# penn-graphics-research/DOT

Measured on AMD Instinct MI355X. Metric: ms_per_time_step, lower is better.
Workload: dtype f64; 1 GPU; bar17K_twist; nV=17315, nT=86058, energy=SNH, subdomains=32, script=twist, parallelism=32 subdomains on 1 GPU

## Files before the change

### dot_amd/csrc/dotmi_api.hip

```cpp
#include "dotmi_handle.hpp"

extern "C" {

int dotmi_set_state(dotmi_handle *h, const double *x, const double *v, const double *x_n)
{
    if (!h || !x || !v) return DOTMI_E_INVALID;
    HIPCHECK(h, hipSetDevice(h->device));
    if (resolve_refresh(h) == DOTMI_E_DEVICE) return DOTMI_E_DEVICE;
    const size_t bytes = sizeof(double) * h->n;
    HIPCHECK(h, hipMemcpyAsync(h->x, x, bytes, hipMemcpyHostToDevice, h->st));
    HIPCHECK(h, hipMemcpyAsync(h->v, v, bytes, hipMemcpyHostToDevice, h->st));
    HIPCHECK(h, hipMemcpyAsync(h->xn, x_n ? x_n : x, bytes, hipMemcpyHostToDevice, h->st));
    HIPCHECK(h, hipStreamSynchronize(h->st));
    std::vector<double> xt(h->n);
    const double *xn_h = x_n ? x_n : x;
    for (int i = 0; i < h->nV; ++i)
        for (int d = 0; d < 3; ++d) {
            const int k = 3 * i + d;
            xt[k] = h->fixed[i] ? xn_h[k] : xn_h[k] + (v[k] * h->dt + h->gdtsq[d]);
        }
    HIPCHECK(h, hipMemcpy(h->xt, xt.data(), bytes, hipMemcpyHostToDevice));
    return 0;
}

// ... 37 lines not shown
    else HIPCHECK(h, hipEventSynchronize(h->evDir));
    memcpy(h->dposPinned, pos, sizeof(double) * 3 * n);
    HIPCHECK(h, hipMemcpyAsync(h->dpos, h->dposPinned, sizeof(double) * 3 * n, hipMemcpyHostToDevice, h->st));
    HIPCHECK(h, hipEventRecord(h->evDir, h->st));
    launch_scatter_rows(n, h->didx, h->dpos, h->x, h->st);
    return 0;
}

int dotmi_refix(dotmi_handle *h, const uint8_t *fixed)
{
    if (!h || !fixed) return DOTMI_E_INVALID;
    HIPCHECK(h, hipSetDevice(h->device));
    if (resolve_refresh(h) == DOTMI_E_DEVICE) return DOTMI_E_DEVICE;
    h->fixed.assign(fixed, fixed + h->nV);
    HIPCHECK(h, hipMemcpy(h->M.fixed, fixed, h->nV, hipMemcpyHostToDevice));
    if (h->pd) return pd_factor(h);
    return refactor(h, h->x, nullptr, nullptr);
}

double dotmi_target_gres(const dotmi_handle *h) { return h ? h->targetGRes : 0.0; }

int dotmi_last_iter_log(const dotmi_handle *h, int32_t cap, double *alpha, double *E, double *g2)
{
    if (!h) return DOTMI_E_INVALID;
    if (h->logPending > 0) {
        dotmi_handle *hm = const_cast<dotmi_handle *>(h);
        const int nlog = h->logPending;
        hm->logPending = 0;
        hm->log_alpha.resize(nlog);
        hm->log_E.resize(nlog);
        hm->log_g2.resize(nlog);
        if (hipSetDevice(h->device) != hipSuccess ||
            hipMemcpy(hm->log_alpha.data(), h->dlog, sizeof(double) * nlog, hipMemcpyDeviceToHost) != hipSuccess ||
// ... 558 lines not shown
```

### dot_amd/csrc/dotmi_create.hip

```cpp
#include "dotmi_handle.hpp"
#include "block_plan.hpp"

namespace dotmi {
std::string g_create_error;
}

namespace dotmi {

void host_features(dotmi_handle *h)
{
    const int nV = h->nV, nT = h->nT;
    h->A.assign((size_t)9 * nT, 0.0);
    h->vol.assign(nT, 0.0);
    h->mass.assign(nV, 0.0);
    for (int e = 0; e < nT; ++e) {
        const int *t = &h->T[4 * e];
        const double *p0 = &h->Xrest[3 * t[0]], *p1 = &h->Xrest[3 * t[1]], *p2 = &h->Xrest[3 * t[2]],
                     *p3 = &h->Xrest[3 * t[3]];
        Mat3 X0;
        for (int i = 0; i < 3; ++i) {
            X0.m[i][0] = p1[i] - p0[i];
            X0.m[i][1] = p2[i] - p0[i];
            X0.m[i][2] = p3[i] - p0[i];
        }
// ... 743 lines not shown
    if (!owner || H.nPatches == 0) return 0;
    for (int p = 0; p < H.nPatches; ++p) {
        const uint16_t *cp = &H.c_ptr[(size_t)p * (H.PO + 1)];
        for (int lv = 0; lv < H.po_cnt[p]; ++lv) {
            const int v = H.pv_gid[(size_t)p * H.PV + lv];
            owner[v] = p;
            if (runlen) runlen[v] = cp[lv + 1] - cp[lv];
        }
    }
    if (elem) std::copy(H.elem.begin(), H.elem.end(), elem);
    if (eown)
        for (size_t s = 0; s < H.eown.size(); ++s) eown[s] = H.eown[s];
    return 0;
}

static int plan_tile_schedule_impl(int32_t nt, const uint8_t *live, const uint8_t *pattern, const int32_t *c0, int32_t eager_min,
                                   int32_t eager_chunk, int64_t *tasks, int64_t *prods, int64_t *n_tasks, int64_t *n_prods,
                                   int64_t *n_levels, int64_t *storage, int64_t *scratch_base, int64_t *row_off, int32_t *row_ld,
                                   const uint8_t *leaf_tile, const int32_t *c0m, const int32_t *ntm, int64_t *row_off_m,
                                   int32_t *row_ld_m)
{
    if (nt < 1 || !live || !pattern || !c0 || !n_tasks || !n_prods) return DOTMI_E_INVALID;
    std::vector<long long> rtOff(nt, -1);
    std::vector<int> rtLd(nt, 0), rtC0(nt, 0);
    long long tot = 0;
    for (int j = 0; j < nt; ++j) {
        if (!live[j]) continue;
        rtC0[j] = 64 * c0[j];
        rtLd[j] = 64 * (j + 1) - rtC0[j];
        rtOff[j] = tot;
// ... 602 lines not shown
        return DOTMI_E_INVALID;
    }
    h->devLoop = !h->gsdd && !h->newton && !h->pd && !h->hi && !(h->flags & (DOTMI_FLAG_HOST_LOOP | DOTMI_FLAG_TIME_PHASES));
    h->earlyBs = h->devLoop && h->tune.earlyBs != 0 &&
                 (h->P.mt_ptr != nullptr || h->P.splitMerge);
    if (h->owner && !(h->earlyBs && h->tune.fuseDir)) {
        h->err = "DOTMI_FLAG_OWNER_EXCHANGE needs the device loop's early order with the fused direction kernel";
        return DOTMI_E_INVALID;
    }
    if (h->earlyBs && h->tune.fuseStep && (!h->shardElems || h->owner)) h->PT.wgCap = h->PTspec.wgCap = 512;
    h->vpFits = false;
    if (h->earlyBs && !h->dist && h->world == 1 && h->tune.fuseStep && h->tune.fuseDir && h->tune.vertexPatches != 0 &&
        (h->mat == DOTMI_ENERGY_SNH || h->tune.vertexPatches > 0) &&
        h->P.ntiles - h->P.ntilesWide + h->P.nquad > 0 && !(h->flags & (DOTMI_FLAG_GSDD | DOTMI_FLAG_NEWTON | DOTMI_FLAG_NEWTON_PCG | DOTMI_FLAG_HOST_LOOP))) {
        const HostVPatches HV = build_vpatches(h->nV, h->nT, h->T.data(), h->Xrest.data(), 512, 85);
        const size_t shm = sizeof(double) * ((size_t)3 * HV.PV + (size_t)3 * HV.RUN) + 2 * (size_t)((HV.PO + 1 + 3) & ~3);
        if (HV.nPatches > 0 && HV.nPatches <= 512 && HV.nPatches <= ELEM_NB_MAX && shm <= 64 * 1024 && HV.PO + 1 <= 256) {
            if (int rc = upload_vpatches(h, HV, h->VP, h->smVP)) return rc;
            h->vpFits = true;
            if (h->tune.fuseLog)
                fprintf(stderr, "dotmi: vertex patches: %d patches, %.2f x the elements, up to %d owned / %d touched vertices, runs %d, %zu B LDS\n",
                        HV.nPatches, (double)h->VP.nSlotsUsed / std::max(1, h->nT), HV.PO, HV.PV, HV.RUN, shm);
        }
    }
    return 0;
}

static int alloc_loop_state(dotmi_handle *h)
{
    if (h->dist) {
        if (int rc = dalloc(h, &h->zstage, (size_t)h->n)) return rc;
        HIPCHECK(h, hipMemsetAsync(h->zstage, 0, sizeof(double) * h->n, h->st));
    }
    if (h->earlyBs) {
        if (int rc = dalloc(h, &h->u_old, (size_t)h->n)) return rc;
        for (int sl = 0; sl <= h->hist; ++sl) {
            if (int rc = dalloc(h, &h->MY[sl], (size_t)h->n)) return rc;
            if (int rc = dalloc(h, &h->HS[sl], (size_t)h->n)) return rc;
        }
    }
    h->logCap = std::min(h->iterCap, 10001) + 1;
    h->kindCap = 4096;
    HIPCHECK(h, hipHostMalloc((void **)&h->h_ctl, sizeof(DevLoop)));
    HIPCHECK(h, hipHostMalloc((void **)&h->h_flags, sizeof(int) * 4));
    HIPCHECK(h, hipMalloc((void **)&h->ctl, sizeof(DevLoop)));
    h->allocs.push_back(h->ctl);
    if (int rc = dalloc(h, &h->dlog, (size_t)3 * h->logCap)) return rc;
// ... 139 lines not shown
```

### dot_amd/csrc/dotmi_devloop.hip

```cpp
#include "dotmi_handle.hpp"

namespace dotmi {

struct Slot {
    int nb = 0;
    const double *spart = nullptr;
    const double *ctlE = nullptr;
};

static int slot_direction(dotmi_handle *h, Slot &s)
{
    if (h->specNow) {
        StepArgs sa{h->p, h->partS, h->alpha_dev, h->alphaMin};
        launch_dirstep(h->M, h->PTspec, h->mat, h->dtSq, h->xt, h->partE, &s.nb, h->Hval, h->z, h->partCT, h->p, h->Hp, h->partS, h->st,
                       h->ctl, sa);
    } else if (h->owner) {
        launch_spmv_zp(h->M, h->HvalOwn, h->z, h->partGC, h->p, h->Hp, h->partS, h->st, h->ctl, 0, -1, h->heldMask, h->ownMask,
                       h->held());
    } else if (h->tune.fuseDir) {
        launch_spmv_zp(h->M, h->Hval, h->z, h->dist ? h->partC : h->partCT, h->p, h->Hp, h->partS, h->st, h->ctl,
                       h->shardElems ? h->v0 : 0, h->shardElems ? h->v1 : -1, nullptr, nullptr, VList(), !h->dist, h->partST);
    } else {
        LbfgsArgs L0;
        memset(&L0, 0, sizeof(L0));
// ... 180 lines not shown
    C.iterCap = h->iterCap;
    C.hist = h->hist;
    C.tol = h->targetGRes;
    C.dtSq = h->dtSq;
    C.x_cur = h->x;
    C.x_trial = h->x_trial;
    C.g_cur = h->g;
    C.g_trial = h->g_trial;
    for (int s = 0; s <= h->hist; ++s) {
        C.S[s] = h->S[s];
        C.Y[s] = h->Y[s];
        C.MY[s] = h->MY[s];
        C.HS[s] = h->HS[s];
    }
    C.u_old = h->u_old;
    devloop_resolve(C);
    C.holdEnable = h->tune.earlyHold ? 1 : 0;
    memcpy(C.predHist, h->predState, sizeof(int) * 2);
    memcpy(&C.predCtr[0][0], h->predState + 2, sizeof(int) * 8);
    memcpy(C.pairCtr, h->pairState, sizeof(int) * 3);
    C.log_alpha = h->dlog;
    C.log_E = h->dlog + h->logCap;
    C.log_g2 = h->dlog + 2 * (size_t)h->logCap;
    C.slot_kind = h->dkind;
    C.logCap = h->logCap;
    C.kindCap = h->kindCap;
    volatile int *flags = h->h_flags;
    flags[0] = 0;
    flags[1] = 0;
    C.notifyFrom = std::max(0, std::min(h->prevSlots - 3, h->prevSlots * 3 / 4));
// ... 222 lines not shown
```

### dot_amd/csrc/dotmi_handle.hpp

```cpp
#pragma once
#include <hip/hip_runtime.h>
#include <rccl/rccl.h>

#include <algorithm>
#include <chrono>
#include <cmath>
#include <cstdio>
#include <cstdlib>
#include <cstring>
#include <functional>
#include <string>
#include <unordered_map>
#include <vector>

#include "../../include/dotmi.h"
#include "dotmi_internal.hpp"
#include "elem_math.hpp"
#include "partition.hpp"
#include "patches.hpp"
#include "vpatches.hpp"


namespace dotmi {

// ... 31 lines not shown
    int tileGroups = -1;
    int tileHfill = 1;
    int tileEagerMin = 0;
    int fastDiag = 1;
    int tileFlow = -1;
    int tileFlowWaitMs = 2000;
    int tileEagerMinRmul = -1;
    bool tileEagerMinRmulByUser = false;
    bool fuseDir = true;
    bool fuseStep = true;
    int pairTrials = -1;
    int vertexPatches = -1;
    int specStep = 0;
    bool earlyHold = true;
    int earlyBs = 2;
    static int geti(const char *name, int dflt)
    {
        const char *ev = getenv(name);
        return ev ? atoi(ev) : dflt;
    }
    static Tuning from_env()
    {
        Tuning t;
        t.wavePacks = geti("DOTMI_WAVE_PACKS", 1) != 0;
        t.tilePasses = std::min(8, std::max(1, geti("DOTMI_TILE_PASSES", 4)));
        t.ndLevels = geti("DOTMI_ND_LEVELS", -1);
        if (t.ndLevels < -1) t.ndLevels = 0;
        t.ndMin = std::max(128, geti("DOTMI_ND_MIN", ND_MIN_SPLIT));
        t.ndMinByUser = getenv("DOTMI_ND_MIN") != nullptr;
        if (const char *ev = getenv("DOTMI_TILE_ROWS")) t.tileRows = std::min(64, std::max(8, atoi(ev) / 8 * 8));
// ... 11 lines not shown
        t.tileGroups = geti("DOTMI_TILE_GROUPS", -1);
        t.tileHfill = geti("DOTMI_TILE_HFILL", 1) != 0;
        t.tileEagerMin = std::max(0, geti("DOTMI_TILE_EAGER_MIN", 0));
        t.tileFlow = geti("DOTMI_TILE_FLOW", -1);
        t.fastDiag = geti("DOTMI_FAST_DIAG", 1);
        t.tileFlowWaitMs = std::max(1, geti("DOTMI_TILE_FLOW_WAIT_MS", 2000));
        t.tileEagerMinRmul = geti("DOTMI_TILE_EAGER_MIN_RMUL", -1);
        t.tileEagerMinRmulByUser = getenv("DOTMI_TILE_EAGER_MIN_RMUL") != nullptr;
        t.earlyBs = geti("DOTMI_EARLY_BACKSOLVE", 2) != 0 ? 2 : 0;
        t.earlyHold = geti("DOTMI_EARLY_HOLD", 1) != 0;
        t.pairTrials = geti("DOTMI_PAIR_TRIALS", -1);
        t.specStep = geti("DOTMI_SPEC_STEP", 0);
        t.vertexPatches = geti("DOTMI_VERTEX_PATCHES", -1);
        t.fuseStep = geti("DOTMI_FUSE_STEP", 1) != 0;
        t.fuseDir = geti("DOTMI_FUSE_DIR", 1) != 0;
        return t;
    }
};

struct dotmi_handle {
    Tuning tune;
#ifdef DOTMI_TEST_HOOKS
    int testIterDelta = 0;
    int testFailRefresh = 0, testRefreshCount = 0;
#endif
    int nV = 0, nT = 0, n = 0, mat = 0, hist = 5, iterCap = 10000;
    double dt = 0, dtSq = 0, grav[3] = {0, 0, 0}, gdtsq[3] = {0, 0, 0}, relTol = 1e-5, alphaMin = 0.1;
    double targetGRes = 0, density = 0;
    int device = 0, rank = 0, world = 1, flags = 0;
    bool dist = false;
// ... 48 lines not shown
    bool tileSplit = false;
    int predState[10] = {0, 0, 1, 1, 1, 1, 1, 1, 1, 1};
    int heldSlots = 0, heldRejected = 0;
    bool tileFlow = false;
    bool fastDiag = false;
    int *tdepPtr = nullptr, *tdepIdx = nullptr, *tdone = nullptr, *tnext = nullptr;
    int tileEpoch = 0, nTtasks = 0, tileFlowWg = 0;
    hipStream_t stDiag = nullptr;
    std::vector<hipEvent_t> tFork, tJoin;
    double tileFlops = 0;
    DevPatches PT, PTall;
    DevPatches PTspec;
    bool specFits = false;
    DevVPatches VP;
    bool vpFits = false, vpNow = false;
    struct SlotMap {
        int *elem = nullptr;
        size_t nSlots = 0;
        double *mu = nullptr, *lam = nullptr;
    };
    SlotMap smAll, smOwn, smSpec, smVP;
    int nOwnElem = 0, v0 = 0, v1 = 0;
    double *x = nullptr, *x_trial = nullptr, *xn = nullptr, *v = nullptr, *xt = nullptr;
    double *g = nullptr, *g_trial = nullptr, *p = nullptr, *q = nullptr, *z = nullptr, *Hp = nullptr;
    double *He = nullptr, *Hval = nullptr, *tmpn = nullptr;
    double *S[HIST_MAX + 1] = {nullptr}, *Y[HIST_MAX + 1] = {nullptr};
    bool refreshPending = false;
    double carryHess = 0, carryFact = 0;
    bool earlyBs = false;
    bool earlyNow = false;
// ... 209 lines not shown
```

### dot_amd/csrc/dotmi_internal.hpp

```cpp
#pragma once
#include <hip/hip_runtime.h>

#include "nd_layout.hpp"
#include "tile_factor.hpp"
#include <stdint.h>

namespace dotmi {

constexpr int HIST_MAX = 6;
inline int elem_wg_cap(int mat) { return mat == 1 ? 768 : 512; }
constexpr int NB_RED = 256;
constexpr int RED_K = 3 * HIST_MAX + 3;
constexpr int BS_WAVE = 256;
constexpr int BS_NARROW = 3072;
constexpr int BS_LONG = 5120;
constexpr int ELEM_NB_MAX = 8192;
constexpr int CHOL_NB = 64;

__host__ __device__ inline size_t hval_idx(int blk, int e) { return (size_t)(blk >> 3) * 72 + (size_t)(8 * e + (blk & 7)); }
inline size_t hval_size(int nnzb) { return (size_t)72 * (((size_t)nnzb + 7) / 8); }

struct DevMesh {
    int nV, nT, nTp;
    int4 *T;
// ... 9 lines not shown

struct DevPatches {
    int nPatches = 0, PE = 0, PV = 0, nSlots = 0, nElem = 0;
    int wgCap = 0;
    ushort4 *tl = nullptr;
    double *A = nullptr;
    double *mu = nullptr, *lam = nullptr, *vol = nullptr;
    double mu0 = 0.0, lam0 = 0.0;
    int *pv_gid = nullptr, *pv_slot = nullptr, *pv_cnt = nullptr;
    unsigned short *c_ptr = nullptr;
    ushort4 *epos = nullptr;
    int2 *pp_rng = nullptr;
    double *gpart = nullptr;
};

struct DevVPatches {
    int nPatches = 0, PE = 0, PV = 0, PO = 0, RUN = 0, nSlotsUsed = 0;
    ushort4 *tl = nullptr, *epos = nullptr;
    double *A = nullptr;
    double *vol = nullptr, *volE = nullptr;
    double *mu = nullptr, *lam = nullptr;
    double mu0 = 0.0, lam0 = 0.0;
    int *pv_gid = nullptr, *pv_cnt = nullptr, *po_cnt = nullptr;
    unsigned short *c_ptr = nullptr;
};
struct ElemVertArgs {
    const double *mass, *xt, *p, *hp;
    const double *spmv_partials;
    const uint8_t *fixed;
    const int *vp_ptr, *vp_off;
    double *rpad;
    double *partE, *partR, *alpha_out;
    double dtSq, alpha_min;
    const double *x0;
    double *g0;
};

struct RowTile {
    long long off;
    int ld, c0;
// ... 143 lines not shown
    int logCap, kindCap;
    int pairNew;
    int abortEpoch;
    int holdEnable, holdNext, holdVerdict;
    int redo;
    int heldSlots, heldRejected;
    int pairSlots, pairRedo;
    int pairCtr[3], pairPad;
    int predHist[2], predCtr[2][4];
    const double *specPartials;
    double alphaMin;
    int specSlots, specRedo, firstTrials, unitFirst;
    double *u_old, *MY[HIST_MAX + 1];
    double *HS[HIST_MAX + 1];
    double *s_new, *y_new, *hs_new;
    double *my_new;
    const double *Lmy[HIST_MAX], *Lhs[HIST_MAX];
};
template <class DL>
__host__ __device__ inline void devloop_resolve(DL &C)
{
    C.s_new = C.S[C.slot];
    C.y_new = C.Y[C.slot];
    C.hs_new = C.HS[C.slot];
    const int m = C.L.m;
    for (int i = 0; i < HIST_MAX; ++i) {
        C.Lmy[i] = i < m ? C.MY[C.order[i]] : nullptr;
        C.Lhs[i] = i < m ? C.HS[C.order[i]] : nullptr;
    }
    C.my_new = m > 0 ? C.MY[C.order[m - 1]] : nullptr;
}
struct VList {
    const int *v = nullptr;
    int n = 0;
};
struct CtlArgs {
    DevLoop *ctl;
    const double *partE, *partR, *alpha_dev;
    int *flags_host;
    int nbE;
    int init;
};

void launch_step_forward(int n, const double *x0, const double *p, double *x, const double *spmv_partials,
                         double alpha_host, int use_partials, double alpha_min, double *alpha_out,
// ... 166 lines not shown
```

### dot_amd/csrc/k_elemvert.hip

```cpp
#include "k_device.hpp"

namespace dotmi {

constexpr int EV_EPT = 2;

#ifdef K_PROFILE
__device__ long long g_evprof[512][8];
extern "C" int dotmi_debug_evprof(long long *out)
{
    return (int)hipMemcpyFromSymbol(out, HIP_SYMBOL(g_evprof), sizeof(long long) * 512 * 8);
}
#define EVSTAMP(i) do { if (threadIdx.x == 0 && blockIdx.x < 512) g_evprof[blockIdx.x][i] = wall_clock64(); } while (0)
#else
#define EVSTAMP(i) do { } while (0)
#endif

template <int MAT, bool PAIR>
__global__ __launch_bounds__(256) void elem_vertex_kernel(DevVPatches VP, ElemVertArgs a, const DevLoop *__restrict__ ctl)
{
    extern __shared__ double lds[];
    __shared__ double sm[4 * RED_K];
    __shared__ double sme[8];
    __shared__ double sh_alpha;
    const bool pairedLaunch = PAIR && a.alpha_min < 0.0;
    const double alphaMin = pairedLaunch ? -a.alpha_min : a.alpha_min;
    const bool second = pairedLaunch && (int)blockIdx.x >= VP.nPatches;
    const int tid = threadIdx.x, p = second ? (int)blockIdx.x - VP.nPatches : (int)blockIdx.x;
    long long t_start = 0;
#ifdef K_PROFILE
    t_start = wall_clock64();
#endif
    const double *__restrict__ x = a.x0;
    double *__restrict__ x_out = nullptr, *__restrict__ g_out = a.g0;
    const double *__restrict__ g_old = nullptr;
    double *__restrict__ s_new = nullptr, *__restrict__ y_new = nullptr, *__restrict__ hs_new = nullptr;
    const double *hs[HIST_MAX], *hy[HIST_MAX];
    int hm = 0, lphase = 1;
    double lalpha = 0.0;
    const bool loop = ctl != nullptr;
    if (loop) {
        const int status = ctl->status;
        lphase = ctl->phase;
        lalpha = ctl->alpha;
        x = ctl->x_cur;
        x_out = ctl->x_trial;
        g_out = ctl->g_trial;
        g_old = ctl->g_cur;
        s_new = ctl->s_new;
        y_new = ctl->y_new;
        hs_new = ctl->hs_new;
        hm = ctl->L.m;
#pragma unroll
        for (int i = 0; i < HIST_MAX; ++i) {
            hs[i] = ctl->L.s[i];
            hy[i] = ctl->L.y[i];
        }
        if (status != 0) return;
    }
#ifdef K_PROFILE
    if (threadIdx.x == 0 && blockIdx.x < 512) g_evprof[blockIdx.x][7] = t_start;
#endif
    EVSTAMP(0);
    double pgv[NB_RED / 64], pHpv[NB_RED / 64];
    const bool usePart = loop && lphase == 0;
    if (usePart && tid < 64) {
#pragma unroll
        for (int u = 0; u < NB_RED / 64; ++u) {
            pgv[u] = a.spmv_partials[tid + 64 * u];
            pHpv[u] = a.spmv_partials[NB_RED + tid + 64 * u];
        }
    }
    constexpr int PE = 256 * EV_EPT;
    double *xs = lds, *gs = lds + 3 * VP.PV;
    unsigned short *cptr = reinterpret_cast<unsigned short *>(gs + 3 * VP.RUN);
    const int nv = VP.pv_cnt[p], no = VP.po_cnt[p];
    const size_t vb = (size_t)p * VP.PV;
    const int gid = tid < VP.PV ? VP.pv_gid[vb + tid] : -1;
    const unsigned short cp_reg = tid <= VP.PO ? VP.c_ptr[(size_t)p * (VP.PO + 1) + tid] : (unsigned short)0;
    const int ov = tid / 3, od = tid - 3 * ov;
    const int ogid_raw = ov < VP.PV ? VP.pv_gid[vb + ov] : -1;
    const bool vlane = tid < 3 * no;
    const int ogid = vlane ? ogid_raw : -1;
    ushort4 tl[EV_EPT], ep[EV_EPT];
    double Ai[EV_EPT][9], mu_[EV_EPT], la_[EV_EPT], vo[EV_EPT], voE[EV_EPT];
    const size_t strideA = (size_t)VP.nPatches * PE;
#pragma unroll
    for (int u = 0; u < EV_EPT; ++u) {
        const size_t s = (size_t)p * PE + u * 256 + tid;
        tl[u] = VP.tl[s];
        ep[u] = VP.epos[s];
#pragma unroll
        for (int k = 0; k < 9; ++k) Ai[u][k] = VP.A[(size_t)k * strideA + s];
        mu_[u] = VP.mu ? VP.mu[s] : VP.mu0;
        la_[u] = VP.mu ? VP.lam[s] : VP.lam0;
        vo[u] = VP.vol[s];
        voE[u] = VP.volE[s];
    }
    double xv[3] = {0, 0, 0}, pv[3] = {0, 0, 0};
    if (gid >= 0) {
#pragma unroll
        for (int d = 0; d < 3; ++d) {
            xv[d] = x[3 * gid + d];
            if (loop) pv[d] = a.p[3 * gid + d];
        }
    }
    const int ok = 3 * ogid + od;
    bool fx = true;
    double gold = 0.0, pk = 0.0, hpk = 0.0, ms = 0.0, xt_own = 0.0, xtv[3] = {0, 0, 0}, si[HIST_MAX], yi[HIST_MAX];
    int cb = 0, ce = 0;
#pragma unroll
    for (int i = 0; i < HIST_MAX; ++i) si[i] = yi[i] = 0.0;
    if (vlane) {
        fx = a.fixed[ogid] != 0;
        ms = a.mass[ogid];
        xt_own = a.xt[ok];
        if (od == 0) {
#pragma unroll
            for (int d = 0; d < 3; ++d) xtv[d] = a.xt[3 * ogid + d];
        }
        cb = a.vp_ptr[ogid];
        ce = a.vp_ptr[ogid + 1];
        if (loop) {
            gold = g_old[ok];
            pk = a.p[ok];
            hpk = a.hp[ok];
#pragma unroll
            for (int i = 0; i < HIST_MAX; ++i) {
// ... 26 lines not shown
                    if (pairedLaunch) a.alpha_out[1] = pair ? al : 0.0;
                }
            } else {
                sh_alpha = al;
                if (p == 0 && loop) *a.alpha_out = al;
            }
        }
    }
    __syncthreads();
    const double alpha = sh_alpha;
    if (second && alpha < 0.0) return;
    EVSTAMP(2);
    if (gid >= 0) {
#pragma unroll
        for (int d = 0; d < 3; ++d) xs[3 * tid + d] = loop ? xv[d] + alpha * pv[d] : xv[d];
    }
    for (int lv = tid + 256; lv < nv; lv += 256) {
        const int g2 = VP.pv_gid[vb + lv];
#pragma unroll
        for (int d = 0; d < 3; ++d) xs[3 * lv + d] = loop ? x[3 * g2 + d] + alpha * a.p[3 * g2 + d] : x[3 * g2 + d];
    }
    __syncthreads();
    EVSTAMP(3);
    constexpr int VC = 4;
    int vof[VC];
#pragma unroll
    for (int c = 0; c < VC; ++c) vof[c] = (cb + c < ce) ? a.vp_off[cb + c] : 0;
    double acc = 0.0;
#pragma unroll
    for (int u = 0; u < EV_EPT; ++u) {
        if (tl[u].x == 0xFFFF) continue;
        const double *p0 = xs + 3 * tl[u].x, *p1 = xs + 3 * tl[u].y, *p2 = xs + 3 * tl[u].z, *p3 = xs + 3 * tl[u].w;
        Mat3 F;
#pragma unroll
        for (int r = 0; r < 3; ++r) {
            const double d0 = p1[r] - p0[r], d1 = p2[r] - p0[r], d2 = p3[r] - p0[r];
#pragma unroll
            for (int c = 0; c < 3; ++c) F.m[r][c] = d0 * Ai[u][c] + d1 * Ai[u][3 + c] + d2 * Ai[u][6 + c];
        }
        const double w = a.dtSq * vo[u];
        double P[3][3];
        if constexpr (MAT == 1) {
// ... 32 lines not shown
        for (int aa = 0; aa < 3; ++aa)
#pragma unroll
            for (int c = 0; c < 3; ++c)
                g[3 + 3 * aa + c] = Ai[u][3 * aa] * P[c][0] + Ai[u][3 * aa + 1] * P[c][1] + Ai[u][3 * aa + 2] * P[c][2];
#pragma unroll
        for (int c = 0; c < 3; ++c) g[c] = -g[3 + c] - g[6 + c] - g[9 + c];
        const int pkk[4] = {ep[u].x, ep[u].y, ep[u].z, ep[u].w};
#pragma unroll
        for (int k = 0; k < 4; ++k)
            if (pkk[k] != 0xFFFF && !second) {
                gs[pkk[k]] = g[3 * k];
                gs[VP.RUN + pkk[k]] = g[3 * k + 1];
                gs[2 * VP.RUN + pkk[k]] = g[3 * k + 2];
            }
    }
    __syncthreads();
    EVSTAMP(4);
    double st[RED_K];
#pragma unroll
    for (int j = 0; j < RED_K; ++j) st[j] = 0.0;
    double ine = 0.0;
    if (vlane && second) {
        if (od == 0) {
            const double dx = xs[3 * ov] - xtv[0], dy = xs[3 * ov + 1] - xtv[1], dz = xs[3 * ov + 2] - xtv[2];
            ine = (dx * dx + dy * dy + dz * dz) * ms / 2.0;
        }
    } else if (vlane) {
        const int kb = cptr[ov], ke = cptr[ov + 1];
        const double *run = gs + od * VP.RUN;
        double sum = 0.0;
        for (int k = kb; k < ke; k += 4) {
            const double w0 = run[k], w1 = k + 1 < ke ? run[k + 1] : 0.0, w2 = k + 2 < ke ? run[k + 2] : 0.0,
                         w3 = k + 3 < ke ? run[k + 3] : 0.0;
            sum += w0;
            if (k + 1 < ke) sum += w1;
            if (k + 2 < ke) sum += w2;
            if (k + 3 < ke) sum += w3;
        }
        const double xt_k = xs[3 * ov + od];
        const double g = fx ? 0.0 : sum + ms * (xt_k - xt_own);
        if (x_out) x_out[ok] = xt_k;
        g_out[ok] = g;
#pragma unroll
        for (int c = 0; c < VC; ++c)
            if (cb + c < ce) a.rpad[vof[c] + od] = -g;
        for (int c = cb + VC; c < ce; ++c) a.rpad[a.vp_off[c] + od] = -g;
        st[0] = g * g;
        if (loop) {
            const double sn = alpha * pk;
            const double yn = g - gold;
            s_new[ok] = sn;
            y_new[ok] = yn;
            hs_new[ok] = alpha * hpk;
            st[1] = yn * sn;
            st[2] = sn * g;
#pragma unroll
            for (int i = 0; i < HIST_MAX; ++i)
                if (i < hm) {
                    st[3 + i] = si[i] * yn;
                    st[3 + HIST_MAX + i] = sn * yi[i];
                    st[3 + 2 * HIST_MAX + i] = si[i] * g;
                }
        }
        if (od == 0) {
            const double dx = xs[3 * ov] - xtv[0], dy = xs[3 * ov + 1] - xtv[1], dz = xs[3 * ov + 2] - xtv[2];
            ine = (dx * dx + dy * dy + dz * dz) * ms / 2.0;
        }
// ... 5 lines not shown
        sme[wv] = we;
        sme[4 + wv] = wi;
    }
    if (!second) write_partials(st, loop ? RED_K : 1, a.partR, sm);
    else __syncthreads();
    if (tid == 0) {
        double *pe = second ? a.partE + 2 * ELEM_NB_MAX : a.partE;
        pe[2 * p] = (sme[0] + sme[1]) + (sme[2] + sme[3]);
        pe[2 * p + 1] = (sme[4] + sme[5]) + (sme[6] + sme[7]);
    }
    EVSTAMP(6);
}

void launch_elem_vertex(const DevVPatches &VP, int mat, const ElemVertArgs &a, hipStream_t st, const DevLoop *ctl)
{
    const size_t shm = sizeof(double) * ((size_t)3 * VP.PV + (size_t)3 * VP.RUN) + 2 * (size_t)((VP.PO + 1 + 3) & ~3);
    const bool paired = ctl && a.alpha_min < 0.0;
    if (paired) {
        if (mat == 0) hipLaunchKernelGGL((elem_vertex_kernel<0, true>), dim3(2 * VP.nPatches), dim3(256), shm, st, VP, a, ctl);
        else hipLaunchKernelGGL((elem_vertex_kernel<1, true>), dim3(2 * VP.nPatches), dim3(256), shm, st, VP, a, ctl);
    } else {
        if (mat == 0) hipLaunchKernelGGL((elem_vertex_kernel<0, false>), dim3(VP.nPatches), dim3(256), shm, st, VP, a, ctl);
        else hipLaunchKernelGGL((elem_vertex_kernel<1, false>), dim3(VP.nPatches), dim3(256), shm, st, VP, a, ctl);
    }
}

}
```

### dot_amd/csrc/vpatches.hpp

```cpp
#pragma once
#include <algorithm>
#include <cstdint>
#include <vector>

#include "patches.hpp"

namespace dotmi {

struct HostVPatches {
    int nPatches = 0, PE = 0, PV = 0, PO = 0, RUN = 0;
    std::vector<int> elem;
    std::vector<uint16_t> tl;
    std::vector<uint16_t> epos;
    std::vector<uint8_t> eown;
    std::vector<int> pv_gid;
    std::vector<int> pv_cnt, po_cnt;
    std::vector<uint16_t> c_ptr;
};

inline HostVPatches build_vpatches(int nV, int nT, const int32_t *T, const double *X, int PE, int maxOwn)
{
    HostVPatches H;
    H.PE = PE;
    double lo[3] = {1e300, 1e300, 1e300}, hi[3] = {-1e300, -1e300, -1e300};
// ... 107 lines not shown
        for (size_t i = 0; i < els[p].size(); ++i) {
            const int e = els[p][i];
            H.elem[eb + i] = e;
            H.eown[eb + i] = owner[T[4 * e]] == p ? 1 : 0;
            for (int k = 0; k < 4; ++k) {
                const int lv = loc[T[4 * e + k]];
                H.tl[(eb + i) * 4 + k] = (uint16_t)lv;
                if (lv < no) H.epos[(eb + i) * 4 + k] = (uint16_t)at[lv]++;
            }
        }
        for (int v : pv) loc[v] = -1;
    }
    return H;
}

}
```

### dot_amd/lib.py

```python
from __future__ import annotations

import ctypes as C
import os

import numpy as np

_HERE = os.path.dirname(os.path.abspath(__file__))
LIB_PATH = os.environ.get("DOTMI_LIBRARY") or os.path.join(_HERE, "libdotmi.so")

c_dp = C.POINTER(C.c_double)
c_ip = C.POINTER(C.c_int32)
c_up = C.POINTER(C.c_uint8)

ENERGY_FCR = 0
ENERGY_SNH = 1
FLAG_TIME_BACKSOLVE = 2
FLAG_FORCE_DIST = 4
FLAG_HOST_LOOP = 8
FLAG_TIME_PHASES = 16
FLAG_GSDD = 32
FLAG_NEWTON = 64
FLAG_ASYNC_REFRESH = 128
FLAG_OWNER_EXCHANGE = 256
FLAG_LBFGS_PD = 512
# ... 30 lines not shown
                ("backsolve_launches", C.c_int64), ("backsolve_stopped", C.c_int64),
                ("backsolve_held", C.c_int64), ("backsolve_held_rejected", C.c_int64),
                ("paired_slots", C.c_int64), ("paired_redone", C.c_int64),
                ("spec_slots", C.c_int64), ("spec_redone", C.c_int64)]


BENCH_KERNELS = ["elem_energy_grad", "elem_energy", "vertex_gather", "spmv_dots", "backsolve", "merge", "build_qpad",
                 "build_p", "step_forward", "elem_hessian", "assemble",
                 "spmv_zp", "merge_early", "elem_step", "gather_early", "dirstep", "elem_vertex"]

EXPORTS = [
    "dotmi_create", "dotmi_destroy", "dotmi_last_error", "dotmi_comm_unique_id", "dotmi_comm_ranks", "dotmi_set_state",
    "dotmi_get_state", "dotmi_set_dirichlet", "dotmi_refix", "dotmi_step", "dotmi_last_iter_log",
    "dotmi_target_gres", "dotmi_eval_energy", "dotmi_eval_gradient", "dotmi_eval_elem_hessians",
    "dotmi_refactor", "dotmi_apply_precond", "dotmi_spmv", "dotmi_get_features", "dotmi_part_size", "dotmi_padded_size",
    "dotmi_part_matrix", "dotmi_factor_storage_bytes", "dotmi_factor_kind", "dotmi_factor_groups", "dotmi_backsolve_form", "dotmi_plan_backsolve_form", "dotmi_probe_direction", "dotmi_bench_precond", "dotmi_bench_energy", "dotmi_bench_kernel", "dotmi_plan_shards", "dotmi_plan_layout", "dotmi_plan_tile_schedule", "dotmi_plan_tile_schedule_two_level", "dotmi_plan_tile_deps", "dotmi_plan_tile_groups", "dotmi_plan_grouped_tile_schedule", "dotmi_plan_tile_fill", "dotmi_plan_tile_fill_mesh", "dotmi_plan_backsolve_tiles", "dotmi_plan_patches", "dotmi_plan_vpatches", "dotmi_plan_rank", "dotmi_partition",
    "dotmi_plan_pd",
    "dotmi_plan_ic", "dotmi_ic_info", "dotmi_ic_factor",
    "dotmi_set_rel_tol", "dotmi_set_time_step", "dotmi_set_lame",
    "dotmi_solve_hessian", "dotmi_set_pcg", "dotmi_pcg_info",
    "dotmi_set_pcg_coarse", "dotmi_pcg_coarse_info", "dotmi_pcg_coarse_matrix", "dotmi_pcg_apply_precond", "dotmi_plan_coarse",
]

_lib = None


class DotmiError(RuntimeError):
    pass


def load() -> C.CDLL:
# ... 45 lines not shown
        L.dotmi_backsolve_form.argtypes = [H]
        L.dotmi_backsolve_form.restype = C.c_int32
    if hasattr(L, "dotmi_factor_kind"):
        L.dotmi_factor_kind.argtypes = [H]
        L.dotmi_factor_kind.restype = C.c_int32
    if hasattr(L, "dotmi_factor_groups"):
        L.dotmi_factor_groups.argtypes = [H]
        L.dotmi_factor_groups.restype = C.c_int32
    L.dotmi_bench_precond.argtypes = [H, C.c_int32, c_dp, C.POINTER(C.c_int64)]
    L.dotmi_bench_energy.argtypes = [H, C.c_int32, c_dp, C.POINTER(C.c_int64)]
    L.dotmi_bench_kernel.argtypes = [H, C.c_int32, C.c_int32, c_dp, C.POINTER(C.c_int64)]
    L.dotmi_plan_shards.argtypes = [C.c_int32, c_ip, C.c_int32, c_ip]
    L.dotmi_plan_rank.argtypes = [C.c_int32, C.c_int32, c_ip, c_ip, C.c_int32, C.c_int32, C.c_int32, c_ip, c_ip, c_ip, c_ip,
                                  c_ip, c_ip, c_ip]
    L.dotmi_partition.argtypes = [C.c_int32, C.c_int32, c_ip, c_dp, C.c_int32, c_ip]
    if hasattr(L, "dotmi_plan_pd"):
        L.dotmi_plan_pd.argtypes = [C.c_int32, C.c_int32, c_ip, c_dp, c_ip, C.POINTER(C.c_int64)]
    if hasattr(L, "dotmi_plan_ic"):
        L.dotmi_plan_ic.argtypes = [C.c_int32, C.c_int32, c_ip] + [c_ip] * 10
        L.dotmi_ic_info.argtypes = [H, c_ip, c_dp, c_ip]
        L.dotmi_ic_factor.argtypes = [H, C.c_int32, c_dp]
    if hasattr(L, "dotmi_solve_hessian"):
        L.dotmi_solve_hessian.argtypes = [H, c_dp, c_dp, C.c_double, C.c_int32, c_ip, c_dp]
        L.dotmi_set_pcg.argtypes = [H, C.c_double, C.c_int32, C.c_int32]
        L.dotmi_pcg_info.argtypes = [H, C.POINTER(C.c_int64), C.POINTER(C.c_int64), c_ip, c_dp]
    if hasattr(L, "dotmi_set_pcg_coarse"):
        L.dotmi_set_pcg_coarse.argtypes = [H, C.c_int32]
        L.dotmi_pcg_coarse_info.argtypes = [H, c_ip, c_ip, c_ip, C.POINTER(C.c_int64)]
        L.dotmi_pcg_coarse_matrix.argtypes = [H, C.c_int32, c_dp]
        L.dotmi_pcg_apply_precond.argtypes = [H, c_dp, c_dp]
# ... 27 lines not shown
```

### include/dotmi.h

```cpp
#ifndef DOTMI_H
#define DOTMI_H

#include <stdint.h>

#ifdef __cplusplus
extern "C" {
#endif

#define DOTMI_ENERGY_FCR 0
#define DOTMI_ENERGY_SNH 1

#define DOTMI_E_INVALID -1
#define DOTMI_E_DEVICE -2
#define DOTMI_E_NOTSPD -3
#define DOTMI_E_NOGPU -4

typedef struct dotmi_handle dotmi_handle;

typedef struct {
    int32_t nV, nT;
    const double *X_rest;
    const int32_t *T;
    const double *mu;
    const double *lambda;
// ... 89 lines not shown
                 dotmi_handle **out);
void dotmi_destroy(dotmi_handle *h);
const char *dotmi_last_error(const dotmi_handle *h);

int dotmi_plan_shards(int32_t nParts, const int32_t *part_scalar_size, int32_t world, int32_t *first_part);

int dotmi_plan_rank(int32_t nV, int32_t nT, const int32_t *T, const int32_t *epart, int32_t nParts, int32_t rank,
                    int32_t world, int32_t *p0, int32_t *p1, int32_t *elems, int32_t *n_elems, int32_t *v0, int32_t *v1,
                    int32_t *part_size);

int dotmi_plan_patches(int32_t nV, int32_t nT, const int32_t *T, const double *X, int32_t PE, int32_t *n_patches, int32_t *pv,
                       int32_t *n_slots, int32_t *elem, uint16_t *tl, uint16_t *epos, int32_t *pv_gid, int32_t *pv_slot,
                       int32_t *pv_cnt, uint16_t *c_ptr, int32_t *pp_rng);
int dotmi_plan_vpatches(int32_t nV, int32_t nT, const int32_t *T, const double *X, int32_t PE, int32_t max_own, int32_t *hdr,
                        int32_t *owner, int32_t *elem, int32_t *eown, int32_t *runlen);
int dotmi_plan_tile_schedule(int32_t nt, const uint8_t *live, const uint8_t *pattern, const int32_t *c0, int32_t eager_min,
                             int32_t eager_chunk, int64_t *tasks, int64_t *prods, int64_t *n_tasks, int64_t *n_prods,
                             int64_t *n_levels, int64_t *storage, int64_t *scratch_base, int64_t *row_off, int32_t *row_ld);
int dotmi_plan_tile_schedule_two_level(int32_t nt, const uint8_t *live, const uint8_t *pattern, const int32_t *c0,
                                       const uint8_t *leaf_tile, const int32_t *c0m, const int32_t *ntm, int32_t eager_min,
                                       int32_t eager_chunk, int64_t *tasks, int64_t *prods, int64_t *n_tasks, int64_t *n_prods,
                                       int64_t *n_levels, int64_t *storage, int64_t *row_off, int32_t *row_ld, int64_t *row_off_m,
                                       int32_t *row_ld_m);
int dotmi_plan_tile_deps(int32_t nt, const uint8_t *live, const uint8_t *pattern, const int32_t *c0, int32_t eager_min,
                         int32_t eager_chunk, int64_t *dep_ptr, int64_t *dep_idx, int64_t *n_deps);
int dotmi_plan_tile_groups(int32_t n_parts, const int64_t *weight, int32_t groups, int32_t *group_of);
int dotmi_plan_grouped_tile_schedule(int32_t n_blocks, int32_t nt, const uint8_t *live, const uint8_t *pattern, int32_t eager_min,
                                     int32_t eager_chunk, int32_t groups, int64_t *tasks, int64_t *n_tasks, int32_t *group_of,
                                     int32_t *group_level, int64_t *clear, int64_t *n_clear, int32_t n_fill, const int32_t *fill_sub,
                                     int32_t *fill_perm, int32_t *fill_start);
// ... 95 lines not shown
```

Baseline: 3.534 ms.

## Pack per-owned-vertex operands into patch records and interleave L-BFGS history pairs

Precomputes a 32-byte record per owned vertex in each vertex patch (mass, fixed flag, scatter count and the first four scatter offsets), so the fused element-vertex kernel reads them with two vector loads instead of gathering from several arrays. L-BFGS s/y history is also stored interleaved per vertex in an extra buffer, so each lane reads one pair per history slot. Search direction and target positions for owned vertices are staged through LDS. This adds LDS use, extra device memory and a second history write, and refix must keep the records in sync.

```diff
diff --git a/dot_amd/csrc/dotmi_api.hip b/dot_amd/csrc/dotmi_api.hip
--- a/dot_amd/csrc/dotmi_api.hip
+++ b/dot_amd/csrc/dotmi_api.hip
@@ -75,9 +75,15 @@
     if (resolve_refresh(h) == DOTMI_E_DEVICE) return DOTMI_E_DEVICE;
     h->fixed.assign(fixed, fixed + h->nV);
     HIPCHECK(h, hipMemcpy(h->M.fixed, fixed, h->nV, hipMemcpyHostToDevice));
+    if (h->VP.orec) {
+        refix_vpatch_records(h->vpRecGid, fixed, h->vpRec);
+        HIPCHECK(h, hipMemcpy(const_cast<VpOwnRec *>(h->VP.orec), h->vpRec.data(), sizeof(VpOwnRec) * h->vpRec.size(), hipMemcpyHostToDevice));
+    }
     if (h->pd) return pd_factor(h);
     return refactor(h, h->x, nullptr, nullptr);
 }
+
+int dotmi_operand_records(const dotmi_handle *h) { return h && h->vpFits ? (h->VP.orec ? 1 : 0) : -1; }
 
 double dotmi_target_gres(const dotmi_handle *h) { return h ? h->targetGRes : 0.0; }
 
diff --git a/dot_amd/csrc/dotmi_create.hip b/dot_amd/csrc/dotmi_create.hip
--- a/dot_amd/csrc/dotmi_create.hip
+++ b/dot_amd/csrc/dotmi_create.hip
@@ -781,6 +781,32 @@
     return 0;
 }
 
+int dotmi_plan_vpatch_records(int32_t nV, int32_t nT, const int32_t *T, const double *X, int32_t PE, int32_t max_own, const double *mass,
+                              const uint8_t *fixed, const int32_t *vp_ptr, const int32_t *vp_off, const uint8_t *fixed2, int32_t *hdr,
+                              int32_t *pv_gid, int32_t *po_cnt, double *rec_mass, int32_t *rec_fixed, int32_t *rec_cnt, int32_t *rec_off)
+{
+    if (nV < 1 || nT < 1 || !T || !X || PE < 1 || max_own < 1 || !mass || !fixed || !vp_ptr || !vp_off || !hdr) return DOTMI_E_INVALID;
+    const HostVPatches H = build_vpatches(nV, nT, T, X, PE, max_own);
+    hdr[0] = H.nPatches;
+    hdr[1] = H.PE;
+    hdr[2] = H.PV;
+    hdr[3] = H.PO;
+    hdr[4] = H.RUN;
+    if (!pv_gid || H.nPatches == 0) return 0;
+    if (!po_cnt || !rec_mass || !rec_fixed || !rec_cnt || !rec_off) return DOTMI_E_INVALID;
+    std::vector<VpOwnRec> R = build_vpatch_records(H, mass, fixed, vp_ptr, vp_off);
+    if (fixed2) refix_vpatch_records(vpatch_own_gid(H), fixed2, R);
+    std::copy(H.pv_gid.begin(), H.pv_gid.end(), pv_gid);
+    std::copy(H.po_cnt.begin(), H.po_cnt.end(), po_cnt);
+    for (size_t i = 0; i < R.size(); ++i) {
+        rec_mass[i] = R[i].mass;
+        rec_fixed[i] = R[i].fixed;
+        rec_cnt[i] = R[i].cnt;
+        for (int c = 0; c < 4; ++c) rec_off[4 * i + c] = R[i].off[c];
+    }
+    return 0;
+}
+
 static int plan_tile_schedule_impl(int32_t nt, const uint8_t *live, const uint8_t *pattern, const int32_t *c0, int32_t eager_min,
                                    int32_t eager_chunk, int64_t *tasks, int64_t *prods, int64_t *n_tasks, int64_t *n_prods,
                                    int64_t *n_levels, int64_t *storage, int64_t *scratch_base, int64_t *row_off, int32_t *row_ld,
@@ -1413,13 +1439,26 @@
         (h->mat == DOTMI_ENERGY_SNH || h->tune.vertexPatches > 0) &&
         h->P.ntiles - h->P.ntilesWide + h->P.nquad > 0 && !(h->flags & (DOTMI_FLAG_GSDD | DOTMI_FLAG_NEWTON | DOTMI_FLAG_NEWTON_PCG | DOTMI_FLAG_HOST_LOOP))) {
         const HostVPatches HV = build_vpatches(h->nV, h->nT, h->T.data(), h->Xrest.data(), 512, 85);
-        const size_t shm = sizeof(double) * ((size_t)3 * HV.PV + (size_t)3 * HV.RUN) + 2 * (size_t)((HV.PO + 1 + 3) & ~3);
+        const bool rec = h->tune.operandRecords != 0 && HV.nPatches > 0 &&
+                         elem_vertex_dyn_lds(HV.PV, HV.RUN, HV.PO, true) + ELEM_VERTEX_STATIC_LDS <= 64 * 1024;
+        const size_t shm = HV.nPatches > 0 ? elem_vertex_dyn_lds(HV.PV, HV.RUN, HV.PO, rec) + ELEM_VERTEX_STATIC_LDS : 0;
         if (HV.nPatches > 0 && HV.nPatches <= 512 && HV.nPatches <= ELEM_NB_MAX && shm <= 64 * 1024 && HV.PO + 1 <= 256) {
             if (int rc = upload_vpatches(h, HV, h->VP, h->smVP)) return rc;
+            if (rec) {
+                std::vector<int> vpp((size_t)h->nV + 1), vpo;
+                HIPCHECK(h, hipMemcpy(vpp.data(), h->P.vp_ptr, sizeof(int) * vpp.size(), hipMemcpyDeviceToHost));
+                vpo.resize((size_t)std::max(vpp[h->nV], 1));
+                HIPCHECK(h, hipMemcpy(vpo.data(), h->P.vp_off, sizeof(int) * (size_t)vpp[h->nV], hipMemcpyDeviceToHost));
+                h->vpRec = build_vpatch_records(HV, h->mass.data(), h->fixed.data(), vpp.data(), vpo.data());
+                h->vpRecGid = vpatch_own_gid(HV);
+                VpOwnRec *d = nullptr;
+                if (int rc = upload(h, &d, h->vpRec)) return rc;
+                h->VP.orec = d;
+            }
             h->vpFits = true;
             if (h->tune.fuseLog)
-                fprintf(stderr, "dotmi: vertex patches: %d patches, %.2f x the elements, up to %d owned / %d touched vertices, runs %d, %zu B LDS\n",
-                        HV.nPatches, (double)h->VP.nSlotsUsed / std::max(1, h->nT), HV.PO, HV.PV, HV.RUN, shm);
+                fprintf(stderr, "dotmi: vertex patches: %d patches, %.2f x the elements, up to %d owned / %d touched vertices, runs %d, %zu B LDS, operand records %s\n",
+                        HV.nPatches, (double)h->VP.nSlotsUsed / std::max(1, h->nT), HV.PO, HV.PV, HV.RUN, shm, rec ? "on" : "off");
         }
     }
     return 0;
@@ -1430,6 +1469,11 @@
     if (h->dist) {
         if (int rc = dalloc(h, &h->zstage, (size_t)h->n)) return rc;
         HIPCHECK(h, hipMemsetAsync(h->zstage, 0, sizeof(double) * h->n, h->st));
+    }
+    if (h->vpFits && h->VP.orec) {
+        const size_t nrec = (size_t)2 * (HIST_MAX + 1) * h->n;
+        if (int rc = dalloc(h, &h->hrec, nrec)) return rc;
+        HIPCHECK(h, hipMemsetAsync(h->hrec, 0, sizeof(double) * nrec, h->st));
     }
     if (h->earlyBs) {
         if (int rc = dalloc(h, &h->u_old, (size_t)h->n)) return rc;
diff --git a/dot_amd/csrc/dotmi_devloop.hip b/dot_amd/csrc/dotmi_devloop.hip
--- a/dot_amd/csrc/dotmi_devloop.hip
+++ b/dot_amd/csrc/dotmi_devloop.hip
@@ -218,6 +218,7 @@
         C.HS[s] = h->HS[s];
     }
     C.u_old = h->u_old;
+    C.hrec = h->hrec;
     devloop_resolve(C);
     C.holdEnable = h->tune.earlyHold ? 1 : 0;
     memcpy(C.predHist, h->predState, sizeof(int) * 2);
diff --git a/dot_amd/csrc/dotmi_handle.hpp b/dot_amd/csrc/dotmi_handle.hpp
--- a/dot_amd/csrc/dotmi_handle.hpp
+++ b/dot_amd/csrc/dotmi_handle.hpp
@@ -69,6 +69,7 @@
     int specStep = 0;
     bool earlyHold = true;
     int earlyBs = 2;
+    int operandRecords = 1;
     static int geti(const char *name, int dflt)
     {
         const char *ev = getenv(name);
@@ -110,6 +111,7 @@
         t.vertexPatches = geti("DOTMI_VERTEX_PATCHES", -1);
         t.fuseStep = geti("DOTMI_FUSE_STEP", 1) != 0;
         t.fuseDir = geti("DOTMI_FUSE_DIR", 1) != 0;
+        t.operandRecords = geti("DOTMI_OPERAND_RECORDS", 1) & 1;
         return t;
     }
 };
@@ -188,6 +190,9 @@
     bool specFits = false;
     DevVPatches VP;
     bool vpFits = false, vpNow = false;
+    std::vector<VpOwnRec> vpRec;
+    std::vector<int> vpRecGid;
+    double *hrec = nullptr;
     struct SlotMap {
         int *elem = nullptr;
         size_t nSlots = 0;
diff --git a/dot_amd/csrc/dotmi_internal.hpp b/dot_amd/csrc/dotmi_internal.hpp
--- a/dot_amd/csrc/dotmi_internal.hpp
+++ b/dot_amd/csrc/dotmi_internal.hpp
@@ -47,6 +47,7 @@
     double *gpart = nullptr;
 };
 
+struct VpOwnRec;
 struct DevVPatches {
     int nPatches = 0, PE = 0, PV = 0, PO = 0, RUN = 0, nSlotsUsed = 0;
     ushort4 *tl = nullptr, *epos = nullptr;
@@ -56,7 +57,13 @@
     double mu0 = 0.0, lam0 = 0.0;
     int *pv_gid = nullptr, *pv_cnt = nullptr, *po_cnt = nullptr;
     unsigned short *c_ptr = nullptr;
-};
+    const VpOwnRec *orec = nullptr;
+};
+inline size_t elem_vertex_dyn_lds(int PV, int RUN, int PO, bool rec)
+{
+    return sizeof(double) * ((size_t)3 * PV + (size_t)3 * RUN + (rec ? (size_t)6 * PO : 0)) + 2 * (size_t)((PO + 1 + 3) & ~3);
+}
+constexpr size_t ELEM_VERTEX_STATIC_LDS = sizeof(double) * (4 * RED_K + 8 + 1);
 struct ElemVertArgs {
     const double *mass, *xt, *p, *hp;
     const double *spmv_partials;
@@ -230,6 +237,8 @@
     double *u_old, *MY[HIST_MAX + 1];
     double *HS[HIST_MAX + 1];
     double *s_new, *y_new, *hs_new;
+    double *hrec, *rec_new;
+    const double *Lrec[HIST_MAX];
     double *my_new;
     const double *Lmy[HIST_MAX], *Lhs[HIST_MAX];
 };
@@ -245,6 +254,8 @@
         C.Lhs[i] = i < m ? C.HS[C.order[i]] : nullptr;
     }
     C.my_new = m > 0 ? C.MY[C.order[m - 1]] : nullptr;
+    C.rec_new = C.hrec ? C.hrec + 6 * C.slot : nullptr;
+    for (int i = 0; i < HIST_MAX; ++i) C.Lrec[i] = (i < m && C.hrec) ? C.hrec + 6 * C.order[i] : nullptr;
 }
 struct VList {
     const int *v = nullptr;
diff --git a/dot_amd/csrc/k_elemvert.hip b/dot_amd/csrc/k_elemvert.hip
--- a/dot_amd/csrc/k_elemvert.hip
+++ b/dot_amd/csrc/k_elemvert.hip
@@ -1,6 +1,9 @@
 #include "k_device.hpp"
+#include "vpatches.hpp"
 
 namespace dotmi {
+
+typedef double ev_pair __attribute__((ext_vector_type(2)));
 
 constexpr int EV_EPT = 2;
 
@@ -15,7 +18,7 @@
 #define EVSTAMP(i) do { } while (0)
 #endif
 
-template <int MAT, bool PAIR>
+template <int MAT, bool PAIR, bool REC>
 __global__ __launch_bounds__(256) void elem_vertex_kernel(DevVPatches VP, ElemVertArgs a, const DevLoop *__restrict__ ctl)
 {
     extern __shared__ double lds[];
@@ -35,6 +38,8 @@
     const double *__restrict__ g_old = nullptr;
     double *__restrict__ s_new = nullptr, *__restrict__ y_new = nullptr, *__restrict__ hs_new = nullptr;
     const double *hs[HIST_MAX], *hy[HIST_MAX];
+    const ev_pair *hr[HIST_MAX];
+    ev_pair *rec_new = nullptr;
     int hm = 0, lphase = 1;
     double lalpha = 0.0;
     const bool loop = ctl != nullptr;
@@ -52,9 +57,14 @@
         hm = ctl->L.m;
 #pragma unroll
         for (int i = 0; i < HIST_MAX; ++i) {
-            hs[i] = ctl->L.s[i];
-            hy[i] = ctl->L.y[i];
-        }
+            if constexpr (REC) {
+                hr[i] = reinterpret_cast<const ev_pair *>(ctl->Lrec[i]);
+            } else {
+                hs[i] = ctl->L.s[i];
+                hy[i] = ctl->L.y[i];
+            }
+        }
+        if constexpr (REC) rec_new = reinterpret_cast<ev_pair *>(ctl->rec_new);
         if (status != 0) return;
     }
 #ifdef K_PROFILE
@@ -72,7 +82,8 @@
     }
     constexpr int PE = 256 * EV_EPT;
     double *xs = lds, *gs = lds + 3 * VP.PV;
-    unsigned short *cptr = reinterpret_cast<unsigned short *>(gs + 3 * VP.RUN);
+    double *po = gs + 3 * VP.RUN, *xo = po + 3 * VP.PO;
+    unsigned short *cptr = reinterpret_cast<unsigned short *>(REC ? xo + 3 * VP.PO : po);
     const int nv = VP.pv_cnt[p], no = VP.po_cnt[p];
     const size_t vb = (size_t)p * VP.PV;
     const int gid = tid < VP.PV ? VP.pv_gid[vb + tid] : -1;
@@ -81,6 +92,15 @@
     const int ogid_raw = ov < VP.PV ? VP.pv_gid[vb + ov] : -1;
     const bool vlane = tid < 3 * no;
     const int ogid = vlane ? ogid_raw : -1;
+    double2 rq0 = make_double2(0.0, 0.0);
+    int4 rq1 = make_int4(0, 0, 0, 0);
+    if constexpr (REC) {
+        if (ov < VP.PO) {
+            const VpOwnRec *r = VP.orec + ((size_t)p * VP.PO + ov);
+            rq0 = *reinterpret_cast<const double2 *>(r);
+            rq1 = *reinterpret_cast<const int4 *>(&r->off[0]);
+        }
+    }
     ushort4 tl[EV_EPT], ep[EV_EPT];
     double Ai[EV_EPT][9], mu_[EV_EPT], la_[EV_EPT], vo[EV_EPT], voE[EV_EPT];
     const size_t strideA = (size_t)VP.nPatches * PE;
@@ -110,7 +130,26 @@
     int cb = 0, ce = 0;
 #pragma unroll
     for (int i = 0; i < HIST_MAX; ++i) si[i] = yi[i] = 0.0;
-    if (vlane) {
+    if constexpr (REC) {
+        if (vlane) {
+            fx = __double2hiint(rq0.y) != 0;
+            ms = rq0.x;
+            ce = __double2loint(rq0.y);
+            xt_own = a.xt[ok];
+            if (loop) {
+                gold = g_old[ok];
+                hpk = a.hp[ok];
+                const size_t rk = (size_t)(3 * (HIST_MAX + 1)) * ogid + od;
+#pragma unroll
+                for (int i = 0; i < HIST_MAX; ++i) {
+                    ev_pair sy = {0.0, 0.0};
+                    if (i < hm) sy = hr[i][rk];
+                    si[i] = sy.x;
+                    yi[i] = sy.y;
+                }
+            }
+        }
+    } else if (vlane) {
         fx = a.fixed[ogid] != 0;
         ms = a.mass[ogid];
         xt_own = a.xt[ok];
@@ -167,6 +206,12 @@
     if (gid >= 0) {
 #pragma unroll
         for (int d = 0; d < 3; ++d) xs[3 * tid + d] = loop ? xv[d] + alpha * pv[d] : xv[d];
+        if constexpr (REC) {
+            if (loop && tid < no) {
+#pragma unroll
+                for (int d = 0; d < 3; ++d) po[3 * tid + d] = pv[d];
+            }
+        }
     }
     for (int lv = tid + 256; lv < nv; lv += 256) {
         const int g2 = VP.pv_gid[vb + lv];
@@ -177,8 +222,15 @@
     EVSTAMP(3);
     constexpr int VC = 4;
     int vof[VC];
-#pragma unroll
-    for (int c = 0; c < VC; ++c) vof[c] = (cb + c < ce) ? a.vp_off[cb + c] : 0;
+    if constexpr (REC) {
+        vof[0] = rq1.x;
+        vof[1] = rq1.y;
+        vof[2] = rq1.z;
+        vof[3] = rq1.w;
+    } else {
+#pragma unroll
+        for (int c = 0; c < VC; ++c) vof[c] = (cb + c < ce) ? a.vp_off[cb + c] : 0;
+    }
     double acc = 0.0;
 #pragma unroll
     for (int u = 0; u < EV_EPT; ++u) {
@@ -241,8 +293,21 @@
                 gs[2 * VP.RUN + pkk[k]] = g[3 * k + 2];
             }
     }
+    if constexpr (REC) {
+        if (vlane) xo[tid] = xt_own;
+    }
     __syncthreads();
     EVSTAMP(4);
+    if constexpr (REC) {
+        if (vlane) {
+            if (loop) pk = po[tid];
+            if (od == 0) {
+                xtv[0] = xt_own;
+                xtv[1] = xo[tid + 1];
+                xtv[2] = xo[tid + 2];
+            }
+        }
+    }
     double st[RED_K];
 #pragma unroll
     for (int j = 0; j < RED_K; ++j) st[j] = 0.0;
@@ -271,13 +336,21 @@
 #pragma unroll
         for (int c = 0; c < VC; ++c)
             if (cb + c < ce) a.rpad[vof[c] + od] = -g;
-        for (int c = cb + VC; c < ce; ++c) a.rpad[a.vp_off[c] + od] = -g;
+        if constexpr (REC) {
+            if (ce > VC) {
+                const int c0 = a.vp_ptr[ogid];
+                for (int c = c0 + VC; c < c0 + ce; ++c) a.rpad[a.vp_off[c] + od] = -g;
+            }
+        } else {
+            for (int c = cb + VC; c < ce; ++c) a.rpad[a.vp_off[c] + od] = -g;
+        }
         st[0] = g * g;
         if (loop) {
             const double sn = alpha * pk;
             const double yn = g - gold;
             s_new[ok] = sn;
             y_new[ok] = yn;
+            if constexpr (REC) rec_new[(size_t)(3 * (HIST_MAX + 1)) * ogid + od] = ev_pair{sn, yn};
             hs_new[ok] = alpha * hpk;
             st[1] = yn * sn;
             st[2] = sn * g;
@@ -313,15 +386,22 @@
 
 void launch_elem_vertex(const DevVPatches &VP, int mat, const ElemVertArgs &a, hipStream_t st, const DevLoop *ctl)
 {
-    const size_t shm = sizeof(double) * ((size_t)3 * VP.PV + (size_t)3 * VP.RUN) + 2 * (size_t)((VP.PO + 1 + 3) & ~3);
+    const bool rec = VP.orec != nullptr;
+    const size_t shm = elem_vertex_dyn_lds(VP.PV, VP.RUN, VP.PO, rec);
     const bool paired = ctl && a.alpha_min < 0.0;
+#define EV_LAUNCH(MATV, PAIRV, NWG)                                                                                          \
+    do {                                                                                                                     \
+        if (rec) hipLaunchKernelGGL((elem_vertex_kernel<MATV, PAIRV, true>), dim3(NWG), dim3(256), shm, st, VP, a, ctl);     \
+        else hipLaunchKernelGGL((elem_vertex_kernel<MATV, PAIRV, false>), dim3(NWG), dim3(256), shm, st, VP, a, ctl);        \
+    } while (0)
     if (paired) {
-        if (mat == 0) hipLaunchKernelGGL((elem_vertex_kernel<0, true>), dim3(2 * VP.nPatches), dim3(256), shm, st, VP, a, ctl);
-        else hipLaunchKernelGGL((elem_vertex_kernel<1, true>), dim3(2 * VP.nPatches), dim3(256), shm, st, VP, a, ctl);
+        if (mat == 0) EV_LAUNCH(0, true, 2 * VP.nPatches);
+        else EV_LAUNCH(1, true, 2 * VP.nPatches);
     } else {
-        if (mat == 0) hipLaunchKernelGGL((elem_vertex_kernel<0, false>), dim3(VP.nPatches), dim3(256), shm, st, VP, a, ctl);
-        else hipLaunchKernelGGL((elem_vertex_kernel<1, false>), dim3(VP.nPatches), dim3(256), shm, st, VP, a, ctl);
-    }
+        if (mat == 0) EV_LAUNCH(0, false, VP.nPatches);
+        else EV_LAUNCH(1, false, VP.nPatches);
+    }
+#undef EV_LAUNCH
 }
 
 }
diff --git a/dot_amd/csrc/vpatches.hpp b/dot_amd/csrc/vpatches.hpp
--- a/dot_amd/csrc/vpatches.hpp
+++ b/dot_amd/csrc/vpatches.hpp
@@ -145,4 +145,42 @@
     return H;
 }
 
+struct VpOwnRec {
+    double mass;
+    int32_t cnt;
+    int32_t fixed;
+    int32_t off[4];
+};
+static_assert(sizeof(VpOwnRec) == 32, "two 16-byte loads per lane");
+
+inline std::vector<VpOwnRec> build_vpatch_records(const HostVPatches &H, const double *mass, const uint8_t *fixed, const int *vp_ptr,
+                                                  const int *vp_off)
+{
+    std::vector<VpOwnRec> R((size_t)H.nPatches * H.PO, VpOwnRec{0.0, 0, 0, {0, 0, 0, 0}});
+    for (int p = 0; p < H.nPatches; ++p)
+        for (int lv = 0; lv < H.po_cnt[p]; ++lv) {
+            const int v = H.pv_gid[(size_t)p * H.PV + lv];
+            VpOwnRec &r = R[(size_t)p * H.PO + lv];
+            r.mass = mass[v];
+            r.fixed = fixed[v] != 0;
+            r.cnt = vp_ptr[v + 1] - vp_ptr[v];
+            for (int c = 0; c < 4 && c < r.cnt; ++c) r.off[c] = vp_off[vp_ptr[v] + c];
+        }
+    return R;
 }
+
+inline std::vector<int> vpatch_own_gid(const HostVPatches &H)
+{
+    std::vector<int> g((size_t)H.nPatches * H.PO, -1);
+    for (int p = 0; p < H.nPatches; ++p)
+        for (int lv = 0; lv < H.po_cnt[p]; ++lv) g[(size_t)p * H.PO + lv] = H.pv_gid[(size_t)p * H.PV + lv];
+    return g;
+}
+
+inline void refix_vpatch_records(const std::vector<int> &own_gid, const uint8_t *fixed, std::vector<VpOwnRec> &R)
+{
+    for (size_t i = 0; i < own_gid.size(); ++i)
+        if (own_gid[i] >= 0) R[i].fixed = fixed[own_gid[i]] != 0;
+}
+
+}
diff --git a/dot_amd/lib.py b/dot_amd/lib.py
--- a/dot_amd/lib.py
+++ b/dot_amd/lib.py
@@ -68,7 +68,7 @@
     "dotmi_get_state", "dotmi_set_dirichlet", "dotmi_refix", "dotmi_step", "dotmi_last_iter_log",
     "dotmi_target_gres", "dotmi_eval_energy", "dotmi_eval_gradient", "dotmi_eval_elem_hessians",
     "dotmi_refactor", "dotmi_apply_precond", "dotmi_spmv", "dotmi_get_features", "dotmi_part_size", "dotmi_padded_size",
-    "dotmi_part_matrix", "dotmi_factor_storage_bytes", "dotmi_factor_kind", "dotmi_factor_groups", "dotmi_backsolve_form", "dotmi_plan_backsolve_form", "dotmi_probe_direction", "dotmi_bench_precond", "dotmi_bench_energy", "dotmi_bench_kernel", "dotmi_plan_shards", "dotmi_plan_layout", "dotmi_plan_tile_schedule", "dotmi_plan_tile_schedule_two_level", "dotmi_plan_tile_deps", "dotmi_plan_tile_groups", "dotmi_plan_grouped_tile_schedule", "dotmi_plan_tile_fill", "dotmi_plan_tile_fill_mesh", "dotmi_plan_backsolve_tiles", "dotmi_plan_patches", "dotmi_plan_vpatches", "dotmi_plan_rank", "dotmi_partition",
+    "dotmi_part_matrix", "dotmi_factor_storage_bytes", "dotmi_factor_kind", "dotmi_factor_groups", "dotmi_backsolve_form", "dotmi_plan_backsolve_form", "dotmi_probe_direction", "dotmi_bench_precond", "dotmi_bench_energy", "dotmi_bench_kernel", "dotmi_plan_shards", "dotmi_plan_layout", "dotmi_plan_tile_schedule", "dotmi_plan_tile_schedule_two_level", "dotmi_plan_tile_deps", "dotmi_plan_tile_groups", "dotmi_plan_grouped_tile_schedule", "dotmi_plan_tile_fill", "dotmi_plan_tile_fill_mesh", "dotmi_plan_backsolve_tiles", "dotmi_plan_patches", "dotmi_plan_vpatches", "dotmi_plan_vpatch_records", "dotmi_operand_records", "dotmi_plan_rank", "dotmi_partition",
     "dotmi_plan_pd",
     "dotmi_plan_ic", "dotmi_ic_info", "dotmi_ic_factor",
     "dotmi_set_rel_tol", "dotmi_set_time_step", "dotmi_set_lame",
@@ -144,6 +144,9 @@
     L.dotmi_plan_rank.argtypes = [C.c_int32, C.c_int32, c_ip, c_ip, C.c_int32, C.c_int32, C.c_int32, c_ip, c_ip, c_ip, c_ip,
                                   c_ip, c_ip, c_ip]
     L.dotmi_partition.argtypes = [C.c_int32, C.c_int32, c_ip, c_dp, C.c_int32, c_ip]
+    if hasattr(L, "dotmi_operand_records"):
+        L.dotmi_operand_records.argtypes = [H]
+        L.dotmi_operand_records.restype = C.c_int32
     if hasattr(L, "dotmi_plan_pd"):
         L.dotmi_plan_pd.argtypes = [C.c_int32, C.c_int32, c_ip, c_dp, c_ip, C.POINTER(C.c_int64)]
     if hasattr(L, "dotmi_plan_ic"):
diff --git a/include/dotmi.h b/include/dotmi.h
--- a/include/dotmi.h
+++ b/include/dotmi.h
@@ -127,6 +127,10 @@
                        int32_t *pv_cnt, uint16_t *c_ptr, int32_t *pp_rng);
 int dotmi_plan_vpatches(int32_t nV, int32_t nT, const int32_t *T, const double *X, int32_t PE, int32_t max_own, int32_t *hdr,
                         int32_t *owner, int32_t *elem, int32_t *eown, int32_t *runlen);
+int dotmi_operand_records(const dotmi_handle *h);
+int dotmi_plan_vpatch_records(int32_t nV, int32_t nT, const int32_t *T, const double *X, int32_t PE, int32_t max_own, const double *mass,
+                              const uint8_t *fixed, const int32_t *vp_ptr, const int32_t *vp_off, const uint8_t *fixed2, int32_t *hdr,
+                              int32_t *pv_gid, int32_t *po_cnt, double *rec_mass, int32_t *rec_fixed, int32_t *rec_cnt, int32_t *rec_off);
 int dotmi_plan_tile_schedule(int32_t nt, const uint8_t *live, const uint8_t *pattern, const int32_t *c0, int32_t eager_min,
                              int32_t eager_chunk, int64_t *tasks, int64_t *prods, int64_t *n_tasks, int64_t *n_prods,
                              int64_t *n_levels, int64_t *storage, int64_t *scratch_base, int64_t *row_off, int32_t *row_ld);
```

Result: faster. 3.499 ms (median of 6 runs) (-1.0%).
